# 10183308/popsift

Measured on AMD Instinct MI355X. Metric: Mpix/s SIFT extract on 1920x1080 (keypoints+descriptors), higher is better.
Workload: dtype f32

## Files before the change

include/popsift_hip.h:

```cpp
#ifndef POPSIFT_HIP_H
#define POPSIFT_HIP_H

#include <stddef.h>
#include <stdint.h>

#ifdef __cplusplus
extern "C" {
#endif

#define POPSIFT_HIP_MAX_OCTAVES 20
#define POPSIFT_HIP_MAX_LEVELS 12
#define POPSIFT_HIP_MAX_BATCH 16
#define POPSIFT_HIP_GAUSS_ALIGN 32
#define POPSIFT_HIP_ORI_MAX 4

typedef enum popsift_hip_status {
    POPSIFT_HIP_OK = 0,
    POPSIFT_HIP_ERR_INVALID = -1,
    POPSIFT_HIP_ERR_DEVICE = -2,
    POPSIFT_HIP_ERR_NO_DEVICE = -3,
    POPSIFT_HIP_ERR_OOM = -4,
    POPSIFT_HIP_ERR_STATE = -5,
    POPSIFT_HIP_ERR_TOO_SMALL = -6
} popsift_hip_status;
// ... 139 lines not shown
#define POPSIFT_HIP_FRAME_SIGMA_MAX 8.0f
int popsift_hip_describe_batch(popsift_hip_ctx* ctx, const void* const* imgs, const popsift_hip_frame* const* frames,
                               const int* n_frames, int n, int kind, int w, int h, int pitch, int ori_mode);

int popsift_hip_wait(popsift_hip_ctx* ctx, int* n_features, int* n_descriptors);
int popsift_hip_fetch(popsift_hip_ctx* ctx, popsift_hip_feature* feats, size_t feats_cap,
                      float* desc, size_t desc_cap);
int popsift_hip_fetch_begin(popsift_hip_ctx* ctx, popsift_hip_feature* feats, size_t feats_cap,
                            float* desc, size_t desc_cap);
int popsift_hip_fetch_end(popsift_hip_ctx* ctx);
int popsift_hip_results_dev(popsift_hip_ctx* ctx, const void** d_feats, const void** d_desc);

int popsift_hip_fetch_item_u8(popsift_hip_ctx* ctx, int k, popsift_hip_feature* feats, size_t feats_cap, uint8_t* desc,
                              size_t desc_cap);
int popsift_hip_fetch_u8(popsift_hip_ctx* ctx, popsift_hip_feature* feats, size_t feats_cap, uint8_t* desc, size_t desc_cap);
int popsift_hip_fetch_begin_item_u8(popsift_hip_ctx* ctx, int k, popsift_hip_feature* feats, size_t feats_cap, uint8_t* desc,
                                    size_t desc_cap);
int popsift_hip_fetch_begin_u8(popsift_hip_ctx* ctx, popsift_hip_feature* feats, size_t feats_cap, uint8_t* desc,
                               size_t desc_cap);
int popsift_hip_results_dev_item_u8(popsift_hip_ctx* ctx, int k, const void** d_feats, const void** d_desc_u8);

void* popsift_hip_host_alloc(size_t bytes);
void  popsift_hip_host_free(void* p);

typedef struct popsift_hip_devfeatures popsift_hip_devfeatures;
int popsift_hip_clone_results(popsift_hip_ctx* ctx, popsift_hip_devfeatures** out);
int popsift_hip_devfeatures_free(popsift_hip_devfeatures* f);
int popsift_hip_devfeatures_info(const popsift_hip_devfeatures* f, int* device, int* n_features, int* n_descriptors);
int popsift_hip_devfeatures_ptrs(const popsift_hip_devfeatures* f, void** d_features, void** d_descriptors,
                                 void** d_reverse_map);
int popsift_hip_devfeatures_alloc(int device, int n_features, int n_descriptors, popsift_hip_devfeatures** out);
int popsift_hip_devfeatures_from_host(int device, const float* desc, int n_descriptors, popsift_hip_devfeatures** out);
int popsift_hip_devfeatures_download(const popsift_hip_devfeatures* f, float* desc, int32_t* rev);
int popsift_hip_devfeatures_download_u8(const popsift_hip_devfeatures* f, uint8_t* desc);

typedef struct popsift_hip_match {
    int32_t best;
    int32_t second;
    int32_t accept;
    float   dist_best;
    float   dist_second;
} popsift_hip_match;
int popsift_hip_match_sets(const popsift_hip_devfeatures* l, const popsift_hip_devfeatures* r, popsift_hip_match* out);
enum { POPSIFT_HIP_MATCH_AUTO = 0, POPSIFT_HIP_MATCH_EXACT = 1, POPSIFT_HIP_MATCH_SCREEN = 2 };
int popsift_hip_match_set_path(int path);

typedef struct popsift_hip_match_opts {
    float   ratio;
    float   max_dist2;
    int32_t cross_check;
    int32_t reserved;
} popsift_hip_match_opts;
typedef struct popsift_hip_pair {
    int32_t l, r;
    float   dist_best, dist_second;
} popsift_hip_pair;
void popsift_hip_default_match_opts(popsift_hip_match_opts* opts);
int  popsift_hip_match_pairs(const popsift_hip_devfeatures* l, const popsift_hip_devfeatures* r,
                             const popsift_hip_match_opts* opts, popsift_hip_pair* pairs, size_t cap, int* n_pairs);

typedef struct popsift_hip_bytefeatures popsift_hip_bytefeatures;
int popsift_hip_bytefeatures_from_host(int device, const uint8_t* desc, int n_descriptors, popsift_hip_bytefeatures** out);
int popsift_hip_bytefeatures_from_set(const popsift_hip_devfeatures* f, popsift_hip_bytefeatures** out);
int popsift_hip_clone_results_u8(popsift_hip_ctx* ctx, int k, popsift_hip_bytefeatures** out);
int popsift_hip_bytefeatures_free(popsift_hip_bytefeatures* f);
int popsift_hip_bytefeatures_info(const popsift_hip_bytefeatures* f, int* device, int* n_descriptors);
int popsift_hip_bytefeatures_download(const popsift_hip_bytefeatures* f, uint8_t* desc, int32_t* rev);
int popsift_hip_match_bytes(const popsift_hip_bytefeatures* l, const popsift_hip_bytefeatures* r, popsift_hip_match* out);
int popsift_hip_match_pairs_bytes(const popsift_hip_bytefeatures* l, const popsift_hip_bytefeatures* r,
                                  const popsift_hip_match_opts* opts, popsift_hip_pair* pairs, size_t cap, int* n_pairs);

int popsift_hip_get_report(const popsift_hip_ctx* ctx, popsift_hip_report* rep);
int popsift_hip_set_profile(popsift_hip_ctx* ctx, int profile);

int popsift_hip_octave_dims(const popsift_hip_ctx* ctx, int octave, int* w, int* h);
int popsift_hip_download_plane(popsift_hip_ctx* ctx, int octave, int kind, int level, float* out);
int popsift_hip_upload_plane(popsift_hip_ctx* ctx, int octave, int kind, int level, const float* in);
int popsift_hip_download_extrema(popsift_hip_ctx* ctx, popsift_hip_extremum* out, size_t cap, int* n);
int popsift_hip_rerun_keypoint_stages(popsift_hip_ctx* ctx);
enum { POPSIFT_HIP_DEBUG_DET_QCAP = 1, POPSIFT_HIP_DEBUG_CAND_CAP = 2, POPSIFT_HIP_DEBUG_OHIST_CAP = 3,
       POPSIFT_HIP_DEBUG_FAIL_ALLOC = 4, POPSIFT_HIP_DEBUG_DESC_ROWS = 5,
       POPSIFT_HIP_DEBUG_KP_WAVES = 7, POPSIFT_HIP_DEBUG_BLUR_PATH = 8, POPSIFT_HIP_DEBUG_BLUR_SEG = 9,
       POPSIFT_HIP_DEBUG_PYR_TAIL = 10, POPSIFT_HIP_DEBUG_DIRECT_PATH = 11,
       POPSIFT_HIP_DEBUG_DESC_CAP = 12, POPSIFT_HIP_DEBUG_SCALE_PATH = 13 };
int popsift_hip_debug_set(popsift_hip_ctx* ctx, int what, int value);

#ifdef __cplusplus
}
#endif
#endif
```

popsift_amd/_capi.py:

```python
import ctypes as C
import os

import numpy as np

_HERE = os.path.dirname(os.path.abspath(__file__))
LIB_PATH = os.environ.get("POPSIFT_HIP_LIB") or os.path.join(_HERE, "libpopsift_hip.so")

MAX_OCTAVES = 20
ORI_MAX = 4

OK = 0
ERR_INVALID, ERR_DEVICE, ERR_NO_DEVICE, ERR_OOM, ERR_STATE, ERR_TOO_SMALL = -1, -2, -3, -4, -5, -6

SIFT_POPSIFT, SIFT_OPENCV, SIFT_VLFEAT = 0, 1, 2
GAUSS_VLFEAT_COMPUTE, GAUSS_VLFEAT_RELATIVE, GAUSS_VLFEAT_RELATIVE_ALL = 0, 1, 2
GAUSS_OPENCV_COMPUTE, GAUSS_FIXED9, GAUSS_FIXED15 = 3, 4, 5
DESC_LOOP, DESC_ILOOP, DESC_GRID, DESC_IGRID, DESC_NOTILE = 0, 1, 2, 3, 4
NORM_ROOTSIFT, NORM_CLASSIC = 0, 1
SCALE_DEFAULT, SCALE_DIRECT = 0, 1


class Params(C.Structure):
    _fields_ = [
        ("octaves", C.c_int32), ("levels", C.c_int32), ("sigma", C.c_float),
# ... 44 lines not shown
    ("xpos", np.float32), ("ypos", np.float32), ("lpos", np.int32),
    ("sigma", np.float32), ("octave", np.int32), ("cell", np.int32),
])
FRAME_DTYPE = np.dtype([
    ("xpos", np.float32), ("ypos", np.float32), ("sigma", np.float32), ("orientation", np.float32),
    ("octave", np.int32), ("level", np.int32),
])
ORI_COMPUTE, ORI_GIVEN = 0, 1
FRAME_SIGMA_MAX = np.float32(8.0)

_vp, _ip = C.c_void_p, C.POINTER(C.c_int)
SYMBOLS = [
    ("popsift_hip_default_params", None, [C.POINTER(Params)]),
    ("popsift_hip_version", C.c_char_p, []),
    ("popsift_hip_strerror", C.c_char_p, [C.c_int]),
    ("popsift_hip_last_error", C.c_char_p, [_vp]),
    ("popsift_hip_device_count", C.c_int, [_ip]),
    ("popsift_hip_get_device_info", C.c_int, [C.c_int, C.POINTER(DeviceInfo)]),
    ("popsift_hip_device_numa_node", C.c_int, [C.c_int, _ip]),
    ("popsift_hip_ctx_create", C.c_int, [C.c_int, C.POINTER(Params), C.POINTER(_vp)]),
    ("popsift_hip_ctx_destroy", C.c_int, [_vp]),
    ("popsift_hip_get_gauss_table", C.c_int, [_vp, _vp, _vp, _vp, _ip]),
    ("popsift_hip_get_gauss_table_abs0", C.c_int, [_vp, _vp, _vp, _vp, _ip]),
    ("popsift_hip_get_gauss_table_dd", C.c_int, [_vp, _vp, _vp, _vp, _ip]),
    ("popsift_hip_submit_u8", C.c_int, [_vp, _vp, C.c_int, C.c_int, C.c_int]),
    ("popsift_hip_submit_f32", C.c_int, [_vp, _vp, C.c_int, C.c_int, C.c_int]),
    ("popsift_hip_submit_dev_u8", C.c_int, [_vp, _vp, C.c_int, C.c_int, C.c_int]),
    ("popsift_hip_submit_dev_f32", C.c_int, [_vp, _vp, C.c_int, C.c_int, C.c_int]),
    ("popsift_hip_submit_pinned_u8", C.c_int, [_vp, _vp, C.c_int, C.c_int, C.c_int]),
    ("popsift_hip_submit_pinned_f32", C.c_int, [_vp, _vp, C.c_int, C.c_int, C.c_int]),
    ("popsift_hip_submit_batch", C.c_int, [_vp, C.POINTER(C.c_void_p), C.c_int, C.c_int, C.c_int, C.c_int, C.c_int]),
    ("popsift_hip_describe_batch", C.c_int, [_vp, C.POINTER(C.c_void_p), C.POINTER(C.c_void_p), C.POINTER(C.c_int), C.c_int,
                                             C.c_int, C.c_int, C.c_int, C.c_int, C.c_int]),
    ("popsift_hip_wait_batch", C.c_int, [_vp, C.POINTER(C.c_int), C.POINTER(C.c_int), C.POINTER(C.c_int)]),
    ("popsift_hip_fetch_item", C.c_int, [_vp, C.c_int, _vp, C.c_size_t, _vp, C.c_size_t]),
    ("popsift_hip_results_dev_item", C.c_int, [_vp, C.c_int, C.POINTER(C.c_void_p), C.POINTER(C.c_void_p)]),
    ("popsift_hip_fetch_begin_item", C.c_int, [_vp, C.c_int, _vp, C.c_size_t, _vp, C.c_size_t]),
    ("popsift_hip_wait", C.c_int, [_vp, _ip, _ip]),
    ("popsift_hip_fetch", C.c_int, [_vp, _vp, C.c_size_t, _vp, C.c_size_t]),
    ("popsift_hip_fetch_begin", C.c_int, [_vp, _vp, C.c_size_t, _vp, C.c_size_t]),
    ("popsift_hip_fetch_end", C.c_int, [_vp]),
    ("popsift_hip_results_dev", C.c_int, [_vp, C.POINTER(_vp), C.POINTER(_vp)]),
    ("popsift_hip_fetch_item_u8", C.c_int, [_vp, C.c_int, _vp, C.c_size_t, _vp, C.c_size_t]),
    ("popsift_hip_fetch_u8", C.c_int, [_vp, _vp, C.c_size_t, _vp, C.c_size_t]),
    ("popsift_hip_fetch_begin_item_u8", C.c_int, [_vp, C.c_int, _vp, C.c_size_t, _vp, C.c_size_t]),
    ("popsift_hip_fetch_begin_u8", C.c_int, [_vp, _vp, C.c_size_t, _vp, C.c_size_t]),
    ("popsift_hip_results_dev_item_u8", C.c_int, [_vp, C.c_int, C.POINTER(C.c_void_p), C.POINTER(C.c_void_p)]),
    ("popsift_hip_host_alloc", _vp, [C.c_size_t]),
    ("popsift_hip_host_free", None, [_vp]),
    ("popsift_hip_clone_results", C.c_int, [_vp, C.POINTER(_vp)]),
    ("popsift_hip_devfeatures_free", C.c_int, [_vp]),
    ("popsift_hip_devfeatures_info", C.c_int, [_vp, _ip, _ip, _ip]),
    ("popsift_hip_devfeatures_ptrs", C.c_int, [_vp, C.POINTER(_vp), C.POINTER(_vp), C.POINTER(_vp)]),
    ("popsift_hip_devfeatures_alloc", C.c_int, [C.c_int, C.c_int, C.c_int, C.POINTER(_vp)]),
    ("popsift_hip_devfeatures_from_host", C.c_int, [C.c_int, _vp, C.c_int, C.POINTER(_vp)]),
    ("popsift_hip_devfeatures_download", C.c_int, [_vp, _vp, _vp]),
    ("popsift_hip_devfeatures_download_u8", C.c_int, [_vp, _vp]),
    ("popsift_hip_match_sets", C.c_int, [_vp, _vp, _vp]),
    ("popsift_hip_match_set_path", C.c_int, [C.c_int]),
    ("popsift_hip_default_match_opts", None, [C.POINTER(MatchOpts)]),
    ("popsift_hip_match_pairs", C.c_int, [_vp, _vp, C.POINTER(MatchOpts), _vp, C.c_size_t, _ip]),
    ("popsift_hip_bytefeatures_from_host", C.c_int, [C.c_int, _vp, C.c_int, C.POINTER(_vp)]),
    ("popsift_hip_bytefeatures_from_set", C.c_int, [_vp, C.POINTER(_vp)]),
    ("popsift_hip_clone_results_u8", C.c_int, [_vp, C.c_int, C.POINTER(_vp)]),
    ("popsift_hip_bytefeatures_free", C.c_int, [_vp]),
    ("popsift_hip_bytefeatures_info", C.c_int, [_vp, _ip, _ip]),
    ("popsift_hip_bytefeatures_download", C.c_int, [_vp, _vp, _vp]),
    ("popsift_hip_match_bytes", C.c_int, [_vp, _vp, _vp]),
    ("popsift_hip_match_pairs_bytes", C.c_int, [_vp, _vp, C.POINTER(MatchOpts), _vp, C.c_size_t, _ip]),
    ("popsift_hip_get_report", C.c_int, [_vp, C.POINTER(Report)]),
    ("popsift_hip_set_profile", C.c_int, [_vp, C.c_int]),
    ("popsift_hip_octave_dims", C.c_int, [_vp, C.c_int, _ip, _ip]),
    ("popsift_hip_download_plane", C.c_int, [_vp, C.c_int, C.c_int, C.c_int, _vp]),
    ("popsift_hip_upload_plane", C.c_int, [_vp, C.c_int, C.c_int, C.c_int, _vp]),
    ("popsift_hip_download_extrema", C.c_int, [_vp, _vp, C.c_size_t, _ip]),
    ("popsift_hip_rerun_keypoint_stages", C.c_int, [_vp]),
    ("popsift_hip_debug_set", C.c_int, [_vp, C.c_int, C.c_int]),
]
MATCH_AUTO, MATCH_EXACT, MATCH_SCREEN = 0, 1, 2
STAGES = ("pyramid", "detect", "refine", "orientation", "scan", "descriptor")
DEBUG_DET_QCAP, DEBUG_CAND_CAP, DEBUG_OHIST_CAP, DEBUG_FAIL_ALLOC, DEBUG_DESC_ROWS, DEBUG_KP_WAVES = 1, 2, 3, 4, 5, 7
DEBUG_BLUR_PATH, DEBUG_BLUR_SEG, DEBUG_PYR_TAIL, DEBUG_DIRECT_PATH, DEBUG_DESC_CAP = 8, 9, 10, 11, 12
DEBUG_SCALE_PATH = 13
MAX_BATCH = 16
IMG_HOST_U8, IMG_HOST_F32, IMG_DEV_U8, IMG_DEV_F32, IMG_PINNED_U8, IMG_PINNED_F32 = range(6)

_lib = None


def _desc_type(fmt):
    if fmt == "f32":
        return np.float32
    if fmt == "u8":
        return np.uint8
    raise ValueError("fmt: 'f32' or 'u8', got %r" % (fmt,))


def quantize_u8(desc):
    d = np.asarray(desc, np.float32)
    with np.errstate(invalid="ignore"):
        pos = d > 0
        t = np.trunc(d)
        r = np.where(np.abs(d - t) >= np.float32(0.5), t + np.float32(1.0), t)
        r = np.where(d >= np.float32(255.0), np.float32(255.0), r)
        r = np.where(pos, r, np.float32(0.0))
    return r.astype(np.uint8)


class PopsiftHipError(RuntimeError):
    def __init__(self, status, where, detail=""):
        self.status = status
        msg = "%s failed: %d (%s)" % (where, status, lib().popsift_hip_strerror(status).decode())
        if detail:
            msg += ": " + detail
        super().__init__(msg)


def lib():
    global _lib
    if _lib is None:
        if not os.path.exists(LIB_PATH):
            raise ImportError(
                "%s not found: build it with `python -c 'import __graft_entry__ as g; g.build()'` "
                "(hipcc --offload-arch=gfx950); there is no CPU fallback" % LIB_PATH)
        L = C.CDLL(LIB_PATH)
        for name, res, args in SYMBOLS:
            fn = getattr(L, name)
            fn.restype = res
            fn.argtypes = args
        _lib = L
    return _lib


def default_params(**kw):
    p = Params()
    lib().popsift_hip_default_params(C.byref(p))
    for k, v in kw.items():
        if not hasattr(p, k):
            raise AttributeError(k)
        setattr(p, k, v)
    return p


def device_count():
    n = C.c_int(0)
    rc = lib().popsift_hip_device_count(C.byref(n))
    return n.value if rc == OK else 0


def device_info(device=0):
    d = DeviceInfo()
    rc = lib().popsift_hip_get_device_info(device, C.byref(d))
    if rc != OK:
        raise PopsiftHipError(rc, "popsift_hip_get_device_info")
    return d


class DevFeatures:

    def __init__(self, handle):
        self._h = handle

    @classmethod
    def from_host(cls, desc, device=0):
        desc = np.ascontiguousarray(desc, np.float32).reshape(-1, 128)
        h = _vp()
# ... 398 lines not shown
```

popsift_amd/csrc/ctx.hip:

```cpp
#include <hip/hip_runtime.h>

#include <algorithm>
#include <atomic>
#include <cmath>
#include <cstdarg>
#include <cstddef>
#include <cstdio>
#include <cstdlib>
#include <cstring>
#include <new>
#include <type_traits>
#include <vector>

#include "devfeatures.h"
#include "kernels.h"
#include "sift_types.h"
#include "trace.h"

using namespace popsift_hip;

namespace {

constexpr int PITCH_ALIGN = 64;
constexpr int PROFILE_REPS = 4;
// ... 22 lines not shown
            p = nullptr;
            cap = 0;
        }
        return e;
    }
};

}

struct ImageSlot {
    DevBuf<char> input;
    void*        h_input = nullptr;
    size_t       h_input_cap = 0;
    DevBuf<float>       arena;
    DevBuf<InitExt>     iext;
    DevBuf<InitExt>     iext2;
    DevBuf<FilterState> fstate;
    DevBuf<int>         fhist;
    DevBuf<Ext>         ext;
    DevBuf<float, PS_ORI_NBINS> ohist;
    DevBuf<popsift_hip_feature> feats;
    DevBuf<float, 128> desc;
    DevBuf<int>        map;
    DevBuf<float2>     rot;
    DevBuf<DescRec>    drec;
    DevBuf<int2>       cand;
    DevBuf<int>        partial;
    DevBuf<int>        ovf;
    bool               sized = false;
    DevBuf<popsift_hip_feature> alt_feats;
    DevBuf<float, 128>          alt_desc;
    bool moved = false;
    DevBuf<uint8_t, 128> desc_u8;
    bool u8_read = false;
    DevBuf<popsift_hip_frame>   frames;
    popsift_hip_frame*          h_frames = nullptr;
    DevBuf<int>                 fcounts, perm, inv;
    DevBuf<popsift_hip_feature> lfeats;
    int n_frames = 0;

    size_t desc_cap() const { return std::min({desc.cap, map.cap, rot.cap, drec.cap}); }

    void release()
    {
        auto each = [](auto&... b) { ((void)b.release(), ...); };
        each(input, arena, iext, iext2, fstate, fhist, ext, ohist, feats, desc, map, rot, drec, cand, partial, ovf, alt_feats,
             alt_desc, desc_u8, frames, fcounts, perm, inv, lfeats);
        if (h_input) (void)hipHostFree(h_input);
        if (h_frames) (void)hipHostFree(h_frames);
    }
};

struct popsift_hip_ctx {
    int                device = 0;
    popsift_hip_params p{};
    int                levels = 3, L = 6;
    GaussRows<POPSIFT_HIP_MAX_LEVELS> tab{};
    GaussRows<POPSIFT_HIP_MAX_LEVELS> abs0{};
    float*             d_abs0 = nullptr;
    int                direct_path = 0;
    GaussRows<POPSIFT_HIP_MAX_OCTAVES> dd{};
    float*             d_dd = nullptr;
    int                scale_path = 0;
    SiftConsts         sc{};
    hipStream_t        stream = nullptr;
    hipEvent_t         ev_begin = nullptr, ev_end = nullptr;
    hipEvent_t         ev_stage[POPSIFT_HIP_STAGE_COUNT + 1] = {};

    int  in_w = 0, in_h = 0;
    int  frozen_octaves = -1;
    bool have_image = false, finished = false;
    bool batch_ok = false;
    int  nb = 1;
    bool describe = false;
    int  ori_given = 0;
    int  frames_max = 0;

    ImageSlot slot[PS_MAX_BATCH];
    BatchDesc bd{};
    PyrDesc   pd{};
    int       kp_waves = 65536;
    int       det_qcap = 1 << 30;
    int       desc_rows = 1 << 30;
    BlurTune  blur_tune{0, 0};
    int       pyr_tail = 0;
    int       cand_cap_init = 1 << 20;
    bool      cand_cap_user = false;
    int       ohist_cap_init = 0;
    int       desc_cap_init = 0;
    size_t    ext_cap = 0;
    int       cand_cap = 0, desc_cap = 0;
    size_t    ohist_cap = 0;
    hipStream_t copy_stream = nullptr;
    hipEvent_t  ev_u8 = nullptr;
    bool     copy_pending = false;
    unsigned long submit_seq = 0, copy_seq = 0;
    Counters* d_ct = nullptr;
    Counters* h_ct = nullptr;
    PyrDesc*  d_pd = nullptr;
    PyrDesc*  h_pd = nullptr;
    int       n_feat[PS_MAX_BATCH] = {}, n_desc[PS_MAX_BATCH] = {};

    int                    fail_alloc_in = 0;
    int                    profile = 0;
    std::vector<EventPair> blur_events;
    size_t                 blur_events_used = 0;
    popsift_hip_report     rep{};

    char err[256] = {0};
};

namespace {

int fail(popsift_hip_ctx* c, int code, const char* fmt, ...)
{
    if (c) {
        va_list ap;
        va_start(ap, fmt);
        vsnprintf(c->err, sizeof(c->err), fmt, ap);
        va_end(ap);
    }
    return code;
}

#define HIP_TRY(c, call)                                                                              \
    do {                                                                                              \
        hipError_t e__ = (call);                                                                      \
        if (e__ != hipSuccess)                                                                        \
            return fail((c), e__ == hipErrorOutOfMemory ? POPSIFT_HIP_ERR_OOM : POPSIFT_HIP_ERR_DEVICE, \
                        "%s:%d %s -> %s", __FILE__, __LINE__, #call, hipGetErrorString(e__));          \
    } while (0)

#ifdef POPSIFT_SYNC_CHECK
#define SYNC_CHK(c, what)                                                                                     \
    do {                                                                                                      \
        hipError_t e__ = hipStreamSynchronize((c)->stream);                                                   \
        if (e__ == hipSuccess) e__ = hipGetLastError();                                                       \
        if (e__ != hipSuccess) {                                                                              \
            fprintf(stderr, "%s:%d sync check after %s: %s\n", __FILE__, __LINE__, what, hipGetErrorString(e__)); \
            return fail((c), POPSIFT_HIP_ERR_DEVICE, "sync check after %s: %s", what, hipGetErrorString(e__)); \
        }                                                                                                     \
    } while (0)
#else
#define SYNC_CHK(c, what) \
    do {                  \
    } while (0)
#endif

int span_for(int gauss_mode, float sigma)
{
    if (gauss_mode == POPSIFT_HIP_GAUSS_OPENCV_COMPUTE) {
        int span = int(roundf(2.0f * 4.0f * sigma + 1.0f)) | 1;
        span >>= 1;
        span += 1;
        return std::min<int>(span, PS_GA - 1);
    }
    return std::min<int>(ceilf(4.0f * sigma) + 1, PS_GA - 1);
}

template <int N>
void compute_filter_rows(GaussRows<N>& t, int gauss_mode)
{
    for (int level = 0; level < N; level++) {
        t.span[level] = std::min(span_for(gauss_mode, t.sigma[level]), PS_GA - 1);
        const float sig = t.sigma[level];
        const int   spn = t.span[level];
        float*      f = &t.filter[level * PS_GA];
        double      sum = 1.0;
        f[0] = 1.0f;
        for (int x = 1; x < spn; x++) {
            const float val = (float)exp(-0.5 * (pow(double(x) / sig, 2.0)));
            f[x] = val;
            sum += 2.0f * val;
        }
        for (int x = 0; x < spn; x++) f[x] = (float)(f[x] / sum);
        for (int x = spn; x < PS_GA; x++) f[x] = 0.0f;
    }
}

void init_tables(popsift_hip_ctx* c)
{
    const popsift_hip_params& p = c->p;
    const float sigma0 = p.sigma;
    const int   levels = c->levels;
    const float initial_blur = p.assume_initial_blur ? p.initial_blur * powf(2.0f, p.upscale_factor) : 0.0f;
    auto&       t = c->tab;
    memset(&t, 0, sizeof(t));
    t.sigma[0] = p.assume_initial_blur ? sqrtf(fabsf(sigma0 * sigma0 - initial_blur * initial_blur)) : sigma0;
    for (int lvl = 1; lvl < c->L; lvl++) {
        const float sigmaP = sigma0 * powf(2.0f, (float)(lvl - 1) / (float)levels);
        const float sigmaS = sigma0 * powf(2.0f, (float)(lvl) / (float)levels);
        t.sigma[lvl] = sqrtf(sigmaS * sigmaS - sigmaP * sigmaP);
    }
    compute_filter_rows(t, p.gauss_mode);
    auto& a0 = c->abs0;
    memset(&a0, 0, sizeof(a0));
    if (p.gauss_mode == POPSIFT_HIP_GAUSS_VLFEAT_RELATIVE_ALL) {
        for (int lvl = 0; lvl < c->L; lvl++) {
            const float sigmaS = sigma0 * powf(2.0f, (float)lvl / (float)levels);
            a0.sigma[lvl] = sqrtf(fabsf(sigmaS * sigmaS - initial_blur * initial_blur));
        }
        compute_filter_rows(a0, p.gauss_mode);
    }
    auto& dd = c->dd;
    memset(&dd, 0, sizeof(dd));
    for (int oct = 0; oct < POPSIFT_HIP_MAX_OCTAVES; oct++) {
        const float oct_sigma = ldexpf(sigma0, oct);
        const float b = sqrtf(fabsf(oct_sigma * oct_sigma - initial_blur * initial_blur));
        dd.sigma[oct] = ldexpf(b, -oct);
    }
    compute_filter_rows(dd, p.gauss_mode);
    SiftConsts& sc = c->sc;
    sc.sigma0 = sigma0;
    sc.sigma_k = powf(2.0f, 1.0f / levels);
    sc.edge_limit = p.edge_limit;
    sc.threshold = p.threshold * 0.5f * 255.0f / levels;
    sc.max_extrema = p.max_extrema;
    sc.norm_multi = p.norm_multi;
    sc.norm_mode = p.norm_mode;
    sc.sift_mode = p.sift_mode;
    sc.grid_size = p.filter_grid_size > 0 ? p.filter_grid_size : 1;
    sc.up_fac_int = (int)p.upscale_factor;
    sc.desc_mode = p.desc_mode;
    sc.filter_max = p.filter_max_extrema;
    sc.filter_mode = p.filter_sorting;
    sc.det_qcap = c->det_qcap;
    sc.desc_rows = c->desc_rows;
}

void plan_dims(const popsift_hip_ctx* c, int w, int h, int octaves_cfg, int* n_oct, int* bw, int* bh)
{
    const float scaleFactor = 1.0f / powf(2.0f, -c->p.upscale_factor);
    int         oct = octaves_cfg;
    if (oct < 0) oct = std::max(int(floorf(logf((float)std::min(w, h)) / logf(2.0f)) - 3.0f + scaleFactor), 1);
    oct = std::min(oct, PS_MAX_OCT);
    *n_oct = oct;
    *bw = (int)ceilf(w * scaleFactor);
    *bh = (int)ceilf(h * scaleFactor);
}

hipError_t ctx_malloc(popsift_hip_ctx* c, void** p, size_t bytes)
{
    if (c->fail_alloc_in > 0 && --c->fail_alloc_in == 0) {
        *p = nullptr;
        return hipErrorOutOfMemory;
    }
    return hipMalloc(p, bytes);
}

template <class T, size_t PER>
int grow(popsift_hip_ctx* c, DevBuf<T, PER>& b, size_t need)
{
    if (need <= b.cap) return 0;
    HIP_TRY(c, b.release());
    HIP_TRY(c, ctx_malloc(c, (void**)&b.p, need * PER * sizeof(T)));
    b.cap = need;
    return 0;
}

void refresh_caps(popsift_hip_ctx* c)
{
    size_t cand = 1 << 30, desc = 1 << 30, hist = (size_t)1 << 40;
    for (int k = 0; k < c->nb; k++) {
        const ImageSlot& s = c->slot[k];
        cand = std::min(cand, s.cand.cap);
        desc = std::min(desc, s.desc_cap());
        hist = std::min(hist, s.ohist.cap);
        Slot& v = c->bd.s[k];
        v.arena = s.arena.p;
        v.ct = c->d_ct + k;
        v.cand = s.cand.p;
        v.ovf = s.ovf.p;
        v.iext = s.iext.p;
        v.iext2 = s.iext2.p;
        v.fstate = s.fstate.p;
        v.fhist = s.fhist.p;
        v.ohist = s.ohist.p;
        v.ext = s.ext.p;
        v.partial = s.partial.p;
        v.map = s.map.p;
        v.rot = s.rot.p;
        v.drec = s.drec.p;
        v.feats = s.feats.p;
        v.desc = s.desc.p;
    }
    c->cand_cap = (int)cand;
    c->desc_cap = (int)desc;
    c->ohist_cap = hist;
}

int slot_desc_cap(popsift_hip_ctx* c, ImageSlot& s, size_t need)
{
    if (need <= s.desc_cap()) return 0;
    HIP_TRY(c, s.desc.release());
    HIP_TRY(c, s.map.release());
    HIP_TRY(c, s.rot.release());
    HIP_TRY(c, s.drec.release());
    if (int rc = grow(c, s.desc, need)) return rc;
    if (int rc = grow(c, s.map, need)) return rc;
    if (int rc = grow(c, s.rot, need)) return rc;
    return grow(c, s.drec, need);
}

template <typename F>
int ensure_cap(popsift_hip_ctx* c, F grow_slot)
{
    int rc = 0;
    for (int k = 0; k < c->nb && !rc; k++) rc = grow_slot(c->slot[k]);
    refresh_caps(c);
    return rc;
// ... 1747 lines not shown
                           hipMemcpyDeviceToHost));
    return POPSIFT_HIP_OK;
}

int popsift_hip_upload_plane(popsift_hip_ctx* c, int octave, int kind, int level, const float* in)
{
    float*         p = nullptr;
    const OctDesc* od = nullptr;
    if (!in) return POPSIFT_HIP_ERR_INVALID;
    if (c && c->have_image && kind == 1 && c->pd.dog_fly)
        return fail(c, POPSIFT_HIP_ERR_STATE, "DoG planes are not stored (params.store_dog = 0): upload Gaussian planes");
    if (int rc = plane_ptr(c, octave, kind, level, &p, &od)) return rc;
    HIP_TRY(c, hipSetDevice(c->device));
    HIP_TRY(c, hipStreamSynchronize(c->stream));
    HIP_TRY(c, hipMemcpy2D(p, (size_t)od->pitch * 4, in, (size_t)od->w * 4, (size_t)od->w * 4, od->h,
                           hipMemcpyHostToDevice));
    return POPSIFT_HIP_OK;
}

int popsift_hip_download_extrema(popsift_hip_ctx* c, popsift_hip_extremum* out, size_t cap, int* n)
{
    if (!c) return POPSIFT_HIP_ERR_INVALID;
    if (int rc = finish(c)) return rc;
    const int total = c->rep.ext_total;
    if (n) *n = total;
    if (!out) return POPSIFT_HIP_OK;
    if (cap < (size_t)total) return fail(c, POPSIFT_HIP_ERR_TOO_SMALL, "output buffer too small");
    HIP_TRY(c, hipSetDevice(c->device));
    std::vector<InitExt> tmp((size_t)std::max(c->sc.max_extrema, 1));
    size_t               k = 0;
    for (int o = 0; o < c->pd.n_oct; o++) {
        const int cnt = c->rep.ext_ct[o];
        if (cnt <= 0) continue;
        HIP_TRY(c, hipMemcpy(tmp.data(), final_iext(c) + (size_t)o * c->sc.max_extrema, (size_t)cnt * sizeof(InitExt),
                             hipMemcpyDeviceToHost));
        for (int i = 0; i < cnt; i++, k++) {
            out[k].xpos = tmp[i].xpos;
            out[k].ypos = tmp[i].ypos;
            out[k].lpos = tmp[i].lpos;
            out[k].sigma = tmp[i].sigma;
            out[k].octave = o;
            out[k].cell = tmp[i].cell;
        }
    }
    return POPSIFT_HIP_OK;
}

int popsift_hip_debug_set(popsift_hip_ctx* c, int what, int value)
{
    if (!c) return POPSIFT_HIP_ERR_INVALID;
    switch (what) {
    case POPSIFT_HIP_DEBUG_DET_QCAP:
        c->det_qcap = c->sc.det_qcap = std::max(value, 0);
        return POPSIFT_HIP_OK;
    case POPSIFT_HIP_DEBUG_CAND_CAP:
        c->cand_cap_init = std::max(value, DET_SUBQ);
        c->cand_cap_user = true;
        return POPSIFT_HIP_OK;
    case POPSIFT_HIP_DEBUG_OHIST_CAP:
        c->ohist_cap_init = std::max(value, 1);
        return POPSIFT_HIP_OK;
    case POPSIFT_HIP_DEBUG_DESC_CAP:
        c->desc_cap_init = std::max(value, 0);
        return POPSIFT_HIP_OK;
    case POPSIFT_HIP_DEBUG_FAIL_ALLOC:
        c->fail_alloc_in = std::max(value, 0);
        return POPSIFT_HIP_OK;
    case POPSIFT_HIP_DEBUG_KP_WAVES:
        c->kp_waves = std::min(std::max(value / 32 * 32, 32), 1 << 20);
        return POPSIFT_HIP_OK;
    case POPSIFT_HIP_DEBUG_BLUR_PATH:
        if (value < 0 || value > 2) return fail(c, POPSIFT_HIP_ERR_INVALID, "BLUR_PATH: 0, 1 or 2");
        c->blur_tune.path = value;
        return POPSIFT_HIP_OK;
    case POPSIFT_HIP_DEBUG_BLUR_SEG:
        c->blur_tune.seg_rows = std::max(value, 0);
        return POPSIFT_HIP_OK;
    case POPSIFT_HIP_DEBUG_PYR_TAIL:
        c->pyr_tail = value;
        return POPSIFT_HIP_OK;
    case POPSIFT_HIP_DEBUG_DESC_ROWS:
        c->desc_rows = c->sc.desc_rows = std::max(value, 4);
        return POPSIFT_HIP_OK;
    case POPSIFT_HIP_DEBUG_DIRECT_PATH:
        if (value < 0 || value > 1) return fail(c, POPSIFT_HIP_ERR_INVALID, "DIRECT_PATH: 0 or 1");
        c->direct_path = value;
        return POPSIFT_HIP_OK;
    case POPSIFT_HIP_DEBUG_SCALE_PATH:
        if (value < 0 || value > 1) return fail(c, POPSIFT_HIP_ERR_INVALID, "SCALE_PATH: 0 or 1");
        c->scale_path = value;
        return POPSIFT_HIP_OK;
    }
    return fail(c, POPSIFT_HIP_ERR_INVALID, "unknown debug switch %d", what);
}

int popsift_hip_rerun_keypoint_stages(popsift_hip_ctx* c)
{
    if (!c) return POPSIFT_HIP_ERR_INVALID;
    if (!c->have_image || !c->batch_ok) return fail(c, POPSIFT_HIP_ERR_STATE, "no image submitted");
    HIP_TRY(c, hipSetDevice(c->device));
    HIP_TRY(c, hipStreamSynchronize(c->stream));
    if (int rc = drain_copy(c)) return rc;
    c->blur_events_used = 0;
    HIP_TRY(c, hipEventRecord(c->ev_begin, c->stream));
    if (int rc = c->describe ? enqueue_describe_stages(c) : enqueue_keypoint_stages(c)) return rc;
    HIP_TRY(c, hipEventRecord(c->ev_end, c->stream));
    c->finished = false;
    for (ImageSlot& sl : c->slot) sl.moved = false;
    return POPSIFT_HIP_OK;
}

}
```

popsift_amd/csrc/keypoint.hip:

```cpp
#include <hip/hip_runtime.h>

#include "kernels.h"
#include "sift_types.h"

namespace popsift_hip {
namespace {

constexpr float F_PI = 3.14159265358979323846f;
constexpr float F_PI2 = 2.0f * 3.14159265358979323846f;
constexpr float            ORI_WINFACTOR = 1.5f;
constexpr float            DESC_MAGNIFY = 3.0f;

typedef unsigned long long fix64;
__device__ __forceinline__ fix64 to_fix(float w) { return (fix64)(unsigned int)(w * 1048576.0f); }
__device__ __forceinline__ float from_fix(fix64 v) { return (float)((double)v * (1.0 / 1048576.0)); }


__device__ __forceinline__ void wave_lds_sync()
{
    __builtin_amdgcn_fence(__ATOMIC_SEQ_CST, "wavefront");
    __builtin_amdgcn_wave_barrier();
}

__device__ __forceinline__ int wave_incl_scan(int v)
// ... 117 lines not shown
                         -3.33329491539e-1f);
    float       r = fmaf(p * z, t, t);
    r = big ? r + 0.7853981633974483f : r;
    r = (ay > ax) ? 1.5707963267948966f - r : r;
    r = (x < 0.0f) ? 3.14159265358979323846f - r : r;
    return (y < 0.0f) ? -r : r;
}

__device__ __forceinline__ void sincos_cr(float ang, float& s, float& c)
{
    const double x = (double)ang;
    const double q = rint(x * 0.63661977236758134308);
    double       r = fma(-q, 1.57079632679489655800e+00, x);
    r = fma(-q, 6.12323399573676603587e-17, r);
    const double z = r * r;
    double       ps = 2.81145725434552075980e-15;
    ps = fma(ps, z, -7.64716373181981647590e-13);
    ps = fma(ps, z, 1.60590438368216145994e-10);
    ps = fma(ps, z, -2.50521083854417187751e-08);
    ps = fma(ps, z, 2.75573192239858906526e-06);
    ps = fma(ps, z, -1.98412698412698412698e-04);
    ps = fma(ps, z, 8.33333333333333333333e-03);
    ps = fma(ps, z, -1.66666666666666666667e-01);
    const double sr = fma(ps * z, r, r);
    double       pc = -1.56192069685862264622e-16;
    pc = fma(pc, z, 4.77947733238738529744e-14);
    pc = fma(pc, z, -1.14707455977297247139e-11);
    pc = fma(pc, z, 2.08767569878680989792e-09);
    pc = fma(pc, z, -2.75573192239858906526e-07);
    pc = fma(pc, z, 2.48015873015873015873e-05);
    pc = fma(pc, z, -1.38888888888888888889e-03);
    pc = fma(pc, z, 4.16666666666666666667e-02);
    pc = fma(pc, z, -0.5);
    const double cr = fma(pc, z, 1.0);
    const int    n = (int)q & 3;
    const double sd = (n & 1) ? cr : sr, cd = (n & 1) ? sr : cr;
    s = (float)((n & 2) ? -sd : sd);
    c = (float)(((n + 1) & 2) ? -cd : cd);
}

__device__ __forceinline__ float octants(float t, float x, float y, float ax, float ay)
{
    const unsigned int sgn = 0x80000000u;
    const float a = __uint_as_float(__float_as_uint(1.0f - t) ^ (__float_as_uint(ax - ay) & sgn));
    const float b = __uint_as_float(__float_as_uint(1.0f + a) ^ (__float_as_uint(x) & sgn));
    return copysignf(2.0f - b, y);
}

__device__ __forceinline__ float atan2_bins(float y, float x)
{
    const float ax = fabsf(x), ay = fabsf(y);
    const float mx = fmaxf(fmaxf(ax, ay), 1e-30f), mn = fminf(ax, ay);
    const float r = mn * __builtin_amdgcn_rcpf(mx);
    const float s = r * r;
    float       p = fmaf(-0.01492126751691103f, s, 0.06703268736600876f);
    p = fmaf(p, s, -0.14823880791664124f);
    p = fmaf(p, s, 0.24642325937747955f);
    p = fmaf(p, s, -0.42350852489471436f);
    p = fmaf(p, s, 1.2732105255126953f);
    return octants(p * r, x, y, ax, ay);
}

__device__ __forceinline__ float atan2_bins9(float y, float x)
{
    const float ax = fabsf(x), ay = fabsf(y);
    const float mx = fmaxf(fmaxf(ax, ay), 1e-30f), mn = fminf(ax, ay);
    const float r = mn * __builtin_amdgcn_rcpf(mx);
    const float s = r * r;
    float       p = fmaf(0.026540832594037056f, s, -0.1084246039390564f);
    p = fmaf(p, s, 0.22938621044158936f);
    p = fmaf(p, s, -0.4205572307109833f);
    p = fmaf(p, s, 1.2730693817138672f);
    return octants(p * r, x, y, ax, ay);
}

typedef float v2f __attribute__((ext_vector_type(2)));
typedef __attribute__((address_space(3))) fix64 lds_fix64;
typedef __attribute__((address_space(3))) unsigned int lds_u32;

#ifndef KP_NW
#define KP_NW 1
#endif
constexpr int ORI_COPIES = 4;

__global__ __launch_bounds__(64 * KP_NW) void k_orientation(const PyrDesc* __restrict__ pdp, BatchDesc bd, SiftConsts sc,
                                                     int filtered, int hist_cap)
{
    const float* __restrict__   arena = bd.s[blockIdx.y].arena;
    Counters* __restrict__      ct = bd.s[blockIdx.y].ct;
    const InitExt* __restrict__ iext = filtered ? bd.s[blockIdx.y].iext2 : bd.s[blockIdx.y].iext;
    float* __restrict__         ohist = bd.s[blockIdx.y].ohist;
    const int n_oct = pdp->n_oct, L = pdp->L;
    constexpr int    NB = PS_ORI_NBINS + 2;
    __shared__ fix64 s_hist[KP_NW][ORI_COPIES][NB];
    const int        wave = threadIdx.x >> 6, lane = threadIdx.x & 63;
    fix64*           hall = &s_hist[wave][0][0];
    fix64*           hist = s_hist[wave][lane & (ORI_COPIES - 1)];

    __shared__ int ps[PS_MAX_OCT + 1];
    if (threadIdx.x == 0) ext_prefix(ct, sc, n_oct, ps);
    __syncthreads();
    const int total = min(ps[n_oct], hist_cap);

    for (XcdSlice sl = xcd_slice<KP_NW>(); sl.more(total); sl.s += sl.step) {
        const int g = sl.index();
        if (g >= total) continue;
        int o = 0;
        while (o + 1 < n_oct && g >= ps[o + 1]) o++;
        o = uniform(o);
        const InitExt  ie = iext[(size_t)o * sc.max_extrema + (g - uniform(ps[o]))];
        const OctDesc* od = &pdp->o[o];
        const int      w = uniform(od->w), h = uniform(od->h), pitch = uniform(od->pitch);
        const int      lvl = uniform(min(max(ie.lpos, 0), L - 1));
        const float*   layer = arena + uniform64(od->data_off + lvl * od->plane_stride);

        for (int k = lane; k < ORI_COPIES * NB; k += 64) hall[k] = 0ull;
        wave_lds_sync();

        const float x = uniformf(ie.xpos), y = uniformf(ie.ypos), sig = uniformf(ie.sigma);
        const float sigw = ORI_WINFACTOR * sig;
        const int   rad = (int)roundf(3.0f * sigw);
        const float factor2 = (-0.5f / (sigw * sigw)) * 1.4426950408889634f;
        const int   sq_thres = rad * rad;
        const int   xmin = max(1, (int)roundf(x) - rad);
        const int   xmax = min(w - 2, (int)roundf(x) + rad);
        const int   ymin = max(1, (int)roundf(y) - rad);
        const int   ymax = min(h - 2, (int)roundf(y) + rad);
        const int   wx = xmax - xmin + 1;
        const int   hy = ymax - ymin + 1;
#ifdef ORI_PROBE_NOLOOP
        const int   loops = 0;
#else
        const int   loops = (wx > 0 && hy > 0) ? wx * hy : 0;
#endif
        const float inv_wx = __builtin_amdgcn_rcpf((float)max(wx, 1));
        const float wxf = (float)wx, xminf = (float)xmin, yminf = (float)ymin, pitch4f = (float)(4 * pitch);
        const float* corner = layer + (size_t)(ymin * pitch + xmin);

        auto coord = [&](int i, float& fx, float& fy, unsigned int& off) {
            const float fi = (float)i;
            const float frow = floorf((fi + 0.5f) * inv_wx);
            const float fcol = fmaf(-frow, wxf, fi);
            fx = fcol + xminf;
            fy = frow + yminf;
            off = (unsigned int)fmaf(frow, pitch4f, fcol * 4.0f);
        };
        auto bin = [&](float fx, float fy, float gdx, float gdy, bool live) {
            const float dx = fx - x;
            const float dy = fy - y;
            const float sq_dist = truncf(dx * dx + dy * dy);
            if (live && sq_dist <= (float)sq_thres) {
                const float wfix = __builtin_amdgcn_sqrtf(fmaf(gdx, gdx, gdy * gdy)) * __builtin_amdgcn_exp2f(fmaf(sq_dist, factor2, 20.0f));
                float fb = fmaf(atan2_bins(gdy, gdx), (float)PS_ORI_NBINS / 8.0f, (float)PS_ORI_NBINS / 2.0f);
                if (fabsf((fb - floorf(fb)) - 0.5f) < 1e-4f) fb = (float)PS_ORI_NBINS * (atan2_acc(gdy, gdx) + F_PI) / F_PI2;
                int bidx;
                asm("v_cvt_rpi_i32_f32 %0, %1" : "=v"(bidx) : "v"(fb));
                atomicAdd(&hist[bidx], (fix64)(unsigned int)wfix);
            }
        };
        float        xa = 0.0f, ya = 0.0f, xb = 0.0f, yb = 0.0f;
        unsigned int oa = 0, ob = 0;
        float        a0 = 0.0f, a1 = 0.0f, a2 = 0.0f, a3 = 0.0f, b0 = 0.0f, b1 = 0.0f, b2 = 0.0f, b3 = 0.0f;
        const Taps   taps(corner, pitch);
        if (loops > 0) {
            coord(min(lane, loops - 1), xa, ya, oa);
            taps.load_b(oa, a0, a1, a2, a3);
        }
        for (int i = lane; i < loops; i += 128) {
            coord(min(i + 64, loops - 1), xb, yb, ob);
            taps.load_b(ob, b0, b1, b2, b3);
            bin(xa, ya, a0 - a1, a2 - a3, true);
            coord(min(i + 128, loops - 1), xa, ya, oa);
            taps.load_b(oa, a0, a1, a2, a3);
            bin(xb, yb, b0 - b1, b2 - b3, i + 64 < loops);
        }
        wave_lds_sync();

        if (lane < PS_ORI_NBINS) {
            fix64 acc = 0ull;
#pragma unroll
            for (int k = 0; k < ORI_COPIES; k++) acc += hall[k * NB + lane] + (lane == 0 ? hall[k * NB + PS_ORI_NBINS] : 0ull);
            ohist[(size_t)g * PS_ORI_NBINS + lane] = from_fix(acc);
        }
        wave_lds_sync();
    }
}

__device__ __forceinline__ float quad_from_prev(float v)
{
    return __int_as_float(__builtin_amdgcn_update_dpp(0, __float_as_int(v), 0x93, 0xf, 0xf, false));
}
__device__ __forceinline__ float quad_from_next(float v)
{
    return __int_as_float(__builtin_amdgcn_update_dpp(0, __float_as_int(v), 0x39, 0xf, 0xf, false));
}
template <int CTRL>
__device__ __forceinline__ int quad_xchg(int v)
{
    return __builtin_amdgcn_update_dpp(0, v, CTRL, 0xf, 0xf, false);
}
__device__ __forceinline__ float div3(float x)
{
    const float r = 0.333333343267440796f;
    const float q = x * r;
    return fmaf(fmaf(-3.0f, q, x), r, q);
}

__device__ __forceinline__ int ori_peaks_quad(const float* __restrict__ hsrc, int j, bool have, float* angle_out)
{
    constexpr int N = PS_ORI_NBINS, M = N / 4;
    float         h[M], t[M];
#pragma unroll
    for (int b = 0; b < M; b++) h[b] = have ? hsrc[M * j + b] : 0.0f;
#pragma unroll
    for (int pass = 0; pass < 3; pass++) {
        {
            const float lft = quad_from_prev(h[M - 1]), rgt = quad_from_next(h[0]);
#pragma unroll
            for (int b = 0; b < M; b++) t[b] = div3(((b == 0 ? lft : h[b - 1]) + h[b]) + (b == M - 1 ? rgt : h[b + 1]));
        }
        {
            const float lft = quad_from_prev(t[M - 1]), rgt = quad_from_next(t[0]);
#pragma unroll
            for (int b = 0; b < M; b++) h[b] = div3(((b == 0 ? lft : t[b - 1]) + t[b]) + (b == M - 1 ? rgt : t[b + 1]));
        }
    }
    float refined[M], yval[M];
    {
        const float lft = quad_from_prev(h[M - 1]), rgt = quad_from_next(h[0]);
#pragma unroll
        for (int b = 0; b < M; b++) {
            const int   bin = M * j + b;
            const int   prev = (bin == 0) ? N - 1 : bin - 1;
            const float hp = (b == 0) ? lft : h[b - 1], hv = h[b], hn = (b == M - 1) ? rgt : h[b + 1];
            bool        predicate = hv > fmaxf(hp, hn);
            const float num = predicate ? 3.0f * hp - 4.0f * hv + 1.0f * hn : 0.0f;
            const float denB = predicate ? 2.0f * (hp - 2.0f * hv + hn) : 1.0f;
            const float newbin = num / denB;
            predicate = (predicate && newbin >= 0.0f && newbin <= 2.0f);
            refined[b] = predicate ? prev + newbin : -1.0f;
            yval[b] = predicate ? -(num * num) / (4.0f * denB) + hp : -INFINITY;
        }
    }
    unsigned int used = 0u;
    float        best0 = 0.0f;
    int          angles = 0;
#pragma unroll
    for (int k = 0; k < POPSIFT_HIP_ORI_MAX; k++) {
        float bv = 0.0f, br = -1.0f;
        int   bi = -1;
#pragma unroll
        for (int b = 0; b < M; b++) {
            const bool take = !((used >> b) & 1u) && (bi < 0 || yval[b] > bv);
            bv = take ? yval[b] : bv;
            br = take ? refined[b] : br;
            bi = take ? M * j + b : bi;
        }
        {
            const float ov = __int_as_float(quad_xchg<0xB1>(__float_as_int(bv))), orf = __int_as_float(quad_xchg<0xB1>(__float_as_int(br)));
// ... 817 lines not shown
```

popsift_amd/csrc/sift_types.h:

```cpp
#pragma once
#include <stdint.h>

#include <hip/hip_vector_types.h>

#include "../../include/popsift_hip.h"

#define PS_MAX_OCT POPSIFT_HIP_MAX_OCTAVES
#define PS_MAX_PLANES (POPSIFT_HIP_MAX_LEVELS + 3)
#define PS_GA POPSIFT_HIP_GAUSS_ALIGN
#define PS_ORI_NBINS 36

struct OctDesc {
    float*  data;
    float*  dog;
    int64_t data_off;
    int64_t dog_off;
    int64_t plane_stride;
    int     w, h, pitch;
    int     tile_begin;
};

struct PyrDesc {
    int     n_oct;
    int     levels;
    int     L;
    int     total_tiles;
    int     dog_fly;
    int     pad_;
    OctDesc o[PS_MAX_OCT];
};

struct SiftConsts {
    float sigma0, sigma_k, edge_limit, threshold;
    int   max_extrema, norm_multi, norm_mode, sift_mode;
    int   grid_size;
    int   up_fac_int;
    int   desc_mode;
    int   det_qcap;
    int   filter_max;
    int   filter_mode;
    int   desc_rows;
};

struct InitExt {
    float xpos, ypos;
    int   lpos;
    float sigma;
    int   cell;
};

struct Ext {
    float xpos, ypos;
    int   lpos;
    float sigma;
    int   octave;
    int   num_ori;
    int   idx_ori;
    float orientation[POPSIFT_HIP_ORI_MAX];
};

struct DescRec {
    float        x, y;
    float        crsbp, srsbp;
    float        ang_bins;
    float        inv_c;
    unsigned int xymin, xymax;
    unsigned int off_lo, off_hi;
    unsigned int misc;
    float        inv_s;
};

static_assert(sizeof(DescRec) == 48, "three 16-byte loads");

struct Counters {
    int ext_ct[PS_MAX_OCT];
    int ori_ct[PS_MAX_OCT];
    int ext_ps[PS_MAX_OCT];
    int ori_ps[PS_MAX_OCT];
    int ext_total;
    int ori_total;
    int pad[2];
    struct {
        int n;
        int pad[31];
    } qcnt[64];
};
#define DET_SUBQ 64

#define PS_MAX_BATCH POPSIFT_HIP_MAX_BATCH
struct FilterState;
struct Slot {
    float*               arena;
    Counters*            ct;
    const void*          input;
    int2*                cand;
    int*                 ovf;
    InitExt*             iext;
    InitExt*             iext2;
    FilterState*         fstate;
    int*                 fhist;
    float*               ohist;
    Ext*                 ext;
    int*                 partial;
    int*                 map;
    float2*              rot;
    DescRec*             drec;
    popsift_hip_feature* feats;
    float*               desc;
};
struct BatchDesc {
    Slot s[PS_MAX_BATCH];
};

#define FILTER_MAX_CELLS 4096
struct FilterState {
    int                active;
    int                newlimit;
    int                pad[2];
    int                new_ct[PS_MAX_OCT];
    int                cell_count[FILTER_MAX_CELLS];
    int                cell_limit[FILTER_MAX_CELLS];
    int                remaining[FILTER_MAX_CELLS];
    int                cell_mode[FILTER_MAX_CELLS];
    unsigned long long prefix[FILTER_MAX_CELLS];
// ... 15 lines not shown
```

Measured before the change: 3654.

## Restrict orientation histogram sampling to circular disc row spans

The orientation kernel now walks only the pixels inside the circular sampling disc instead of the full bounding square. Each lane computes one row's clipped span, and a wave prefix scan packs the spans into a compact row table in LDS. Sample indices are mapped back to row and column through that table. This drops roughly a fifth of the loads and predicated-off bin work, at the cost of per-batch scan and sync overhead, a serial row-advance loop inside coord, and a new debug knob for the rows per batch.

```diff
diff --git a/include/popsift_hip.h b/include/popsift_hip.h
--- a/include/popsift_hip.h
+++ b/include/popsift_hip.h
@@ -245,7 +245,8 @@
        POPSIFT_HIP_DEBUG_FAIL_ALLOC = 4, POPSIFT_HIP_DEBUG_DESC_ROWS = 5,
        POPSIFT_HIP_DEBUG_KP_WAVES = 7, POPSIFT_HIP_DEBUG_BLUR_PATH = 8, POPSIFT_HIP_DEBUG_BLUR_SEG = 9,
        POPSIFT_HIP_DEBUG_PYR_TAIL = 10, POPSIFT_HIP_DEBUG_DIRECT_PATH = 11,
-       POPSIFT_HIP_DEBUG_DESC_CAP = 12, POPSIFT_HIP_DEBUG_SCALE_PATH = 13 };
+       POPSIFT_HIP_DEBUG_DESC_CAP = 12, POPSIFT_HIP_DEBUG_SCALE_PATH = 13,
+       POPSIFT_HIP_DEBUG_ORI_ROWS = 14 };
 int popsift_hip_debug_set(popsift_hip_ctx* ctx, int what, int value);
 
 #ifdef __cplusplus
diff --git a/popsift_amd/_capi.py b/popsift_amd/_capi.py
--- a/popsift_amd/_capi.py
+++ b/popsift_amd/_capi.py
@@ -150,6 +150,7 @@
 DEBUG_DET_QCAP, DEBUG_CAND_CAP, DEBUG_OHIST_CAP, DEBUG_FAIL_ALLOC, DEBUG_DESC_ROWS, DEBUG_KP_WAVES = 1, 2, 3, 4, 5, 7
 DEBUG_BLUR_PATH, DEBUG_BLUR_SEG, DEBUG_PYR_TAIL, DEBUG_DIRECT_PATH, DEBUG_DESC_CAP = 8, 9, 10, 11, 12
 DEBUG_SCALE_PATH = 13
+DEBUG_ORI_ROWS = 14
 MAX_BATCH = 16
 IMG_HOST_U8, IMG_HOST_F32, IMG_DEV_U8, IMG_DEV_F32, IMG_PINNED_U8, IMG_PINNED_F32 = range(6)
 
diff --git a/popsift_amd/csrc/ctx.hip b/popsift_amd/csrc/ctx.hip
--- a/popsift_amd/csrc/ctx.hip
+++ b/popsift_amd/csrc/ctx.hip
@@ -128,6 +128,7 @@
     int       kp_waves = 65536;
     int       det_qcap = 1 << 30;
     int       desc_rows = 1 << 30;
+    int       ori_rows = 1 << 30;
     BlurTune  blur_tune{0, 0};
     int       pyr_tail = 0;
     int       cand_cap_init = 1 << 20;
@@ -272,6 +273,7 @@
     sc.filter_mode = p.filter_sorting;
     sc.det_qcap = c->det_qcap;
     sc.desc_rows = c->desc_rows;
+    sc.ori_rows = c->ori_rows;
 }
 
 void plan_dims(const popsift_hip_ctx* c, int w, int h, int octaves_cfg, int* n_oct, int* bw, int* bh)
@@ -2185,6 +2187,9 @@
     case POPSIFT_HIP_DEBUG_DESC_ROWS:
         c->desc_rows = c->sc.desc_rows = std::max(value, 4);
         return POPSIFT_HIP_OK;
+    case POPSIFT_HIP_DEBUG_ORI_ROWS:
+        c->ori_rows = c->sc.ori_rows = std::max(value, 4);
+        return POPSIFT_HIP_OK;
     case POPSIFT_HIP_DEBUG_DIRECT_PATH:
         if (value < 0 || value > 1) return fail(c, POPSIFT_HIP_ERR_INVALID, "DIRECT_PATH: 0 or 1");
         c->direct_path = value;
diff --git a/popsift_amd/csrc/keypoint.hip b/popsift_amd/csrc/keypoint.hip
--- a/popsift_amd/csrc/keypoint.hip
+++ b/popsift_amd/csrc/keypoint.hip
@@ -223,6 +223,7 @@
 #define KP_NW 1
 #endif
 constexpr int ORI_COPIES = 4;
+constexpr int ORI_MAXROWS = 64;
 
 __global__ __launch_bounds__(64 * KP_NW) void k_orientation(const PyrDesc* __restrict__ pdp, BatchDesc bd, SiftConsts sc,
                                                      int filtered, int hist_cap)
@@ -234,9 +235,13 @@
     const int n_oct = pdp->n_oct, L = pdp->L;
     constexpr int    NB = PS_ORI_NBINS + 2;
     __shared__ fix64 s_hist[KP_NW][ORI_COPIES][NB];
+    __shared__ unsigned int s_rows[KP_NW][ORI_MAXROWS + 2];
     const int        wave = threadIdx.x >> 6, lane = threadIdx.x & 63;
     fix64*           hall = &s_hist[wave][0][0];
     fix64*           hist = s_hist[wave][lane & (ORI_COPIES - 1)];
+    unsigned int*    rinfo = s_rows[wave];
+    const unsigned int rbase32 = (unsigned int)(size_t)(lds_u32*)rinfo;
+    const int        maxrows_cfg = min(max(sc.ori_rows, 4), ORI_MAXROWS);
 
     __shared__ int ps[PS_MAX_OCT + 1];
     if (threadIdx.x == 0) ext_prefix(ct, sc, n_oct, ps);
@@ -265,32 +270,20 @@
         const int   sq_thres = rad * rad;
         const int   xmin = max(1, (int)roundf(x) - rad);
         const int   xmax = min(w - 2, (int)roundf(x) + rad);
-        const int   ymin = max(1, (int)roundf(y) - rad);
+        const int   ymin0 = max(1, (int)roundf(y) - rad);
         const int   ymax = min(h - 2, (int)roundf(y) + rad);
         const int   wx = xmax - xmin + 1;
-        const int   hy = ymax - ymin + 1;
-#ifdef ORI_PROBE_NOLOOP
-        const int   loops = 0;
-#else
-        const int   loops = (wx > 0 && hy > 0) ? wx * hy : 0;
-#endif
-        const float inv_wx = __builtin_amdgcn_rcpf((float)max(wx, 1));
-        const float wxf = (float)wx, xminf = (float)xmin, yminf = (float)ymin, pitch4f = (float)(4 * pitch);
-        const float* corner = layer + (size_t)(ymin * pitch + xmin);
-
-        auto coord = [&](int i, float& fx, float& fy, unsigned int& off) {
-            const float fi = (float)i;
-            const float frow = floorf((fi + 0.5f) * inv_wx);
-            const float fcol = fmaf(-frow, wxf, fi);
-            fx = fcol + xminf;
-            fy = frow + yminf;
-            off = (unsigned int)fmaf(frow, pitch4f, fcol * 4.0f);
-        };
-        auto bin = [&](float fx, float fy, float gdx, float gdy, bool live) {
+        const int   hy_all = ymax - ymin0 + 1;
+        const float r2 = (float)(sq_thres + 1);
+        const float xminf = (float)xmin, yminf = (float)ymin0, pitch4f = (float)(4 * pitch);
+        const float* corner = layer + (size_t)(ymin0 * pitch + xmin);
+        const int   maxrows = wx <= 255 ? maxrows_cfg : 1;
+
+        auto bin = [&](float fx, float fy, float gdx, float gdy) {
             const float dx = fx - x;
             const float dy = fy - y;
             const float sq_dist = truncf(dx * dx + dy * dy);
-            if (live && sq_dist <= (float)sq_thres) {
+            if (sq_dist <= (float)sq_thres) {
                 const float wfix = __builtin_amdgcn_sqrtf(fmaf(gdx, gdx, gdy * gdy)) * __builtin_amdgcn_exp2f(fmaf(sq_dist, factor2, 20.0f));
                 float fb = fmaf(atan2_bins(gdy, gdx), (float)PS_ORI_NBINS / 8.0f, (float)PS_ORI_NBINS / 2.0f);
                 if (fabsf((fb - floorf(fb)) - 0.5f) < 1e-4f) fb = (float)PS_ORI_NBINS * (atan2_acc(gdy, gdx) + F_PI) / F_PI2;
@@ -299,23 +292,84 @@
                 atomicAdd(&hist[bidx], (fix64)(unsigned int)wfix);
             }
         };
-        float        xa = 0.0f, ya = 0.0f, xb = 0.0f, yb = 0.0f;
-        unsigned int oa = 0, ob = 0;
-        float        a0 = 0.0f, a1 = 0.0f, a2 = 0.0f, a3 = 0.0f, b0 = 0.0f, b1 = 0.0f, b2 = 0.0f, b3 = 0.0f;
-        const Taps   taps(corner, pitch);
-        if (loops > 0) {
-            coord(min(lane, loops - 1), xa, ya, oa);
-            taps.load_b(oa, a0, a1, a2, a3);
-        }
-        for (int i = lane; i < loops; i += 128) {
-            coord(min(i + 64, loops - 1), xb, yb, ob);
-            taps.load_b(ob, b0, b1, b2, b3);
-            bin(xa, ya, a0 - a1, a2 - a3, true);
-            coord(min(i + 128, loops - 1), xa, ya, oa);
-            taps.load_b(oa, a0, a1, a2, a3);
-            bin(xb, yb, b0 - b1, b2 - b3, i + 64 < loops);
-        }
-        wave_lds_sync();
+        const Taps taps(corner, pitch);
+
+        for (int rb = 0; rb < hy_all && wx > 0; rb += maxrows) {
+            const int hy = min(hy_all - rb, maxrows);
+
+            int len = 0, jlo = xmin;
+            if (lane < hy) {
+                const float dy = (float)(ymin0 + rb + lane) - y;
+                const float q = r2 - dy * dy;
+                if (q > 0.0f) {
+                    const float hw = sqrtf(fmaf(r2, 9.5367431640625e-07f, q));
+                    jlo = max(xmin, (int)floorf(x - hw - 1e-3f) + 1);
+                    const int jhi = min(xmax, (int)ceilf(x + hw + 1e-3f) - 1);
+                    len = max(jhi - jlo + 1, 0);
+                    if (len == 0) jlo = xmin;
+                }
+            }
+            const int incl = wave_incl_scan(len);
+            const int start = incl - len;
+            if (lane < hy) rinfo[lane] = (unsigned int)start | ((unsigned int)(start - (jlo - xmin)) << 16);
+            const unsigned long long live = __ballot(len > 0);
+            const int T = __builtin_amdgcn_readlane(incl, 63);
+            const int grow = live != 0ull ? __ffsll((long long)live) - 1 : 0;
+            if (lane == 0) {
+                rinfo[hy] = (unsigned int)T | 0x7fff0000u;
+                rinfo[hy + 1] = 0xffffu;
+            }
+            wave_lds_sync();
+
+#ifdef ORI_PROBE_NOLOOP
+            const int steps = 0;
+#else
+            const int steps = (T + 63) >> 6;
+#endif
+            unsigned int rp = rbase32 + 4u * (unsigned int)grow;
+            float        fr = (float)(rb + grow);
+            unsigned int cur = 0;
+            unsigned int nxt = 0x7fff0000u | 0xffffu;
+            if (T > 0) {
+                cur = rinfo[grow];
+                nxt = rinfo[grow + 1];
+            }
+            auto coord = [&](int i, float& fx, float& fy, unsigned int& off) {
+                while (i >= (int)(nxt & 0xffffu)) {
+                    fr += 1.0f;
+                    rp += 4u;
+                    cur = nxt;
+                    nxt = *(lds_u32*)(size_t)(rp + 4u);
+                }
+                const float fc = (float)(i - ((int)cur >> 16));
+                fx = fc + xminf;
+                fy = fr + yminf;
+                asm("v_cvt_u32_f32 %0, %1" : "=v"(off) : "v"(fmaf(fr, pitch4f, fc * 4.0f)));
+            };
+            float        xa = 0.0f, ya = 0.0f, xb = 0.0f, yb = 0.0f;
+            unsigned int oa = 0, ob = 0;
+            float        a0 = 0.0f, a1 = 0.0f, a2 = 0.0f, a3 = 0.0f, b0 = 0.0f, b1 = 0.0f, b2 = 0.0f, b3 = 0.0f;
+            if (steps > 0) {
+                coord(lane, xa, ya, oa);
+                taps.load_b(oa, a0, a1, a2, a3);
+            }
+            int t = steps, i = lane;
+            for (; t > 2; t -= 2, i += 128) {
+                coord(i + 64, xb, yb, ob);
+                taps.load_b(ob, b0, b1, b2, b3);
+                bin(xa, ya, a0 - a1, a2 - a3);
+                coord(i + 128, xa, ya, oa);
+                taps.load_b(oa, a0, a1, a2, a3);
+                bin(xb, yb, b0 - b1, b2 - b3);
+            }
+            if (t == 2) {
+                coord(i + 64, xb, yb, ob);
+                taps.load_b(ob, b0, b1, b2, b3);
+            }
+            if (t > 0) bin(xa, ya, a0 - a1, a2 - a3);
+            if (t == 2) bin(xb, yb, b0 - b1, b2 - b3);
+            wave_lds_sync();
+        }
 
         if (lane < PS_ORI_NBINS) {
             fix64 acc = 0ull;
diff --git a/popsift_amd/csrc/sift_types.h b/popsift_amd/csrc/sift_types.h
--- a/popsift_amd/csrc/sift_types.h
+++ b/popsift_amd/csrc/sift_types.h
@@ -40,6 +40,7 @@
     int   filter_max;
     int   filter_mode;
     int   desc_rows;
+    int   ori_rows;
 };
 
 struct InitExt {
```

Result: no change. 3651 (-0.1%).
